# floswald/SMM.jl

Measured on AMD Instinct MI355X. Metric: chain-evals/sec (whole node), serialNormal 2p/2m, 4096 chains x 200 iters, higher is better.
Workload: dtype f64

## Files before the change

smm.jl_amd/csrc/smm_chain_persist_loc.hpp:

```cpp
#pragma once
constexpr int PL_LOCN = NORM_CT + CONE_GCAP + 2;
constexpr uint32_t PL_PBASE = ((16u * PL_LOCN + 127u) & ~127u);
constexpr int PL_HASH = 1024;
constexpr size_t PL_TSW_BASE = (size_t)8 * 8192;
constexpr int PL_TSW_TILES = 2048, PL_TSW = 8;
constexpr size_t PL_LATE_BASE = PL_TSW_BASE + (size_t)PL_TSW_TILES * (NORM_WG / 64) * PL_TSW;
constexpr int PL_LATE_N = 16384;
static_assert(PL_LATE_BASE + PL_LATE_N <= (size_t)8 * 60000, "the stamp buffer: the exchange kernels' words start at 8 * 60000");

__host__ __device__ inline size_t persist_loc_smem_bytes(const int np) {
    const size_t hw = (size_t)((H_PARAMS + 2 * np + 1) & ~1);
    const size_t dbl = (size_t)NORM_CT * np + (size_t)np * 8 * NORM_CT + (size_t)NORM_CT * persist_line(np) + 2 * 64 * (size_t)(1 + 2 * np) +
                       2 * NORM_CT * hw + (size_t)PR_ZR * 64 + 16 + 16 + 2 * 64 * 2 + (size_t)PL_LOCN * np + (size_t)PL_LOCN +
                       (size_t)(NORM_WG / 64) * PL_TSW;
    return (size_t)PL_PBASE + 2 * (size_t)CONE_LEVELS * 64 * 4 + 2 * (size_t)CONE_GCAP * 2 + 4 * 16 * 4 + 2 * (size_t)PL_HASH * 4 + dbl * 8;
}

template <int NP>
struct PersistLocLds {
    using L = NormLayout<NP>;
    static constexpr int CT = NORM_CT, RW = L::RW, HW = L::HW, LW = PR_STW + RW, RNGW = 1 + 2 * NP;
    uint32_t pbase, gbase, hbase, tbase;
    uint32_t* s_hdr;
    double *s_theta, *s_part, *s_st, *s_rng, *s_hrow, *s_xrow, *s_z0, *s_const, *s_gth, *s_thr;
    uint4* s_donor;
    unsigned long long *s_ts, *s_wts;
    unsigned* s_arrived; int* s_minprog; unsigned* s_abort; unsigned* s_xmask; int* s_glready; int* s_pub; int* s_hready;
    __device__ inline PersistLocLds(unsigned char* lds) {
        pbase = PL_PBASE;
        gbase = pbase + 2u * CONE_LEVELS * 64 * 4;
        hbase = gbase + 2u * CONE_GCAP * 2;
        tbase = hbase + 4u * 16 * 4;
        s_hdr = (uint32_t*)(lds + hbase);
        s_theta = (double*)(lds + tbase + 2u * PL_HASH * 4);
        s_part = s_theta + CT * NP;
        s_st = s_part + NP * 8 * CT;
        s_rng = s_st + CT * LW;
        s_hrow = s_rng + 2 * 64 * RNGW;
        s_xrow = s_hrow + CT * HW;
        s_z0 = s_xrow + CT * HW;
        s_const = s_z0 + PR_ZR * 64;
        s_ts = (unsigned long long*)(s_const + 16);
        s_arrived = (unsigned*)(s_ts + 8);
        s_minprog = (int*)(s_arrived + 1);
        s_abort = s_arrived + 2;
        s_xmask = s_arrived + 3;
        s_glready = (int*)(s_arrived + 4);
        s_pub = (int*)(s_arrived + 5);
        s_hready = (int*)(s_arrived + 6);
        s_donor = (uint4*)(s_const + 16 + 16);
        s_gth = s_const + 16 + 16 + 2 * 64 * 2;
        s_thr = s_gth + PL_LOCN * NP;
        s_wts = (unsigned long long*)(s_thr + PL_LOCN);
    }
};

__device__ inline uint32_t pl_hslot(const uint32_t chain) { return (chain * 2654435761u) >> 22; }
static_assert(PL_HASH == 1024, "pl_hslot: 10 bits");
__device__ inline void pl_hash_put(uint32_t* tab, const uint32_t chain, const uint32_t local) {
    uint32_t h = pl_hslot(chain);
    while (atomicCAS(&tab[h], 0u, ((chain + 1u) << 16) | local) != 0u) h = (h + 1u) & (PL_HASH - 1);
}
__device__ inline uint32_t pl_hash_get(const uint32_t* tab, const uint32_t chain) {
    uint32_t h = pl_hslot(chain);
    for (int probe = 0; probe < PL_HASH; ++probe) {
        const uint32_t v = tab[h];
        if ((v >> 16) == chain + 1u) return v & 0xffffu;
        if (v == 0u) break;
        h = (h + 1u) & (PL_HASH - 1);
    }
    return 0xffffu;
}

__device__ inline void pl_wts_add(unsigned long long* w, const unsigned long long a, const unsigned long long b, const unsigned long long c,
                                  const unsigned long long d) {
    w[0] += a; w[1] += b; w[2] += c; w[3] += d; w[5] += 1ull;
}
__device__ inline void pl_wts_out(unsigned long long* ts, const unsigned long long* w, const int tile, const int wave) {
    if (tile >= PL_TSW_TILES) return;
    unsigned long long* o = ts + PL_TSW_BASE + ((size_t)tile * (NORM_WG / 64) + (size_t)wave) * PL_TSW;
    for (int k = 0; k < PL_TSW; ++k) o[k] = k == 4 ? (unsigned long long)__builtin_amdgcn_s_getreg((31 << 11) | 4) : w[k];
}

struct PersistLocWalkValues {
    PrWait W; const uint4* ring; const uint16_t* gl; uint32_t c0g; uint32_t tag; int RW; int NPV; int t;
    __device__ __forceinline__ double value(const uint32_t s) const {
        const uint32_t g = s < (uint32_t)NORM_CT ? c0g + s : (uint32_t)gl[s - NORM_CT];
        return pr_tie_value(W, ring, nullptr, tag, RW, NPV, t, g);
    }
};

struct PlGather3 { uint4 q0, q1, q2; };
__device__ __attribute__((noinline)) PlGather3 pl_wait_gather3(const PrWait W, const uint4* p0, const uint4* p1, const uint4* p2, const uint32_t tag, const int t, const int g) {
    PlGather3 o;
    o.q0 = make_uint4(0u, 0u, 0u, 0u); o.q1 = o.q0; o.q2 = o.q0;
    if (*W.s_abort) return o;
    const unsigned long long w0 = wall_clock64();
    unsigned spins = 0;
    for (;;) {
        __builtin_amdgcn_s_sleep(2);
        p2p_u32x4 q0, q1, q2;
        asm volatile("global_load_dwordx4 %0, %3, off sc0 sc1\n\tglobal_load_dwordx4 %1, %4, off sc0 sc1\n\tglobal_load_dwordx4 %2, %5, off sc0 sc1\n\ts_waitcnt vmcnt(0)"
                     : "=&v"(q0), "=&v"(q1), "=&v"(q2) : "v"(p0), "v"(p1), "v"(p2) : "memory");
        o.q0 = make_uint4(q0.x, q0.y, q0.z, q0.w); o.q1 = make_uint4(q1.x, q1.y, q1.z, q1.w); o.q2 = make_uint4(q2.x, q2.y, q2.z, q2.w);
        if (p2p_ll_ok(o.q0, tag) && p2p_ll_ok(o.q1, tag) && p2p_ll_ok(o.q2, tag)) break;
        if ((++spins & 63u) == 0u && pr_give_up(W, w0)) { pr_abort(W, t, g); break; }
    }
    return o;
}

template <int NP, bool WIDE, bool SH, bool PCT = false>
__global__ __launch_bounds__(NORM_WG, 4) void k_chain_persist_loc(const PersistArgs A) {
    static_assert(!PCT || (WIDE && !SH), "thresholds by chain: the wide walk of a single shard");
    static_assert(NP == 1 || NP == 2, "one moment per half of the workgroup");
    extern __shared__ __attribute__((aligned(16))) unsigned char lds[];
    using LY = PersistLocLds<NP>;
    constexpr int CT = NORM_CT, RW = LY::RW, HW = LY::HW, LW = LY::LW, RNGW = LY::RNGW;
    constexpr int NPC = RW / 2, NPH = HW / 2;
    constexpr uint32_t SB = WIDE ? 16u : 8u;
    const int tid = (int)threadIdx.x, lane = tid & 63;
    const int wave = __builtin_amdgcn_readfirstlane(tid >> 6);
    const int tile = (int)blockIdx.x, tiles = (int)gridDim.x;
    const int N = A.N;
    const LY Y(lds);
    const uint32_t epoch = A.epoch;
    const int t0 = A.t0, t1 = A.t1;
    unsigned char* const mine = A.self;
    uint32_t* const pr_ctl = (uint32_t*)(mine + A.o_ctl);
    uint32_t* const pr_progress = (uint32_t*)(mine + A.o_progress);
    const PrWait W{A.err, pr_ctl, Y.s_abort, A.epoch, A.tmo};
    const int rmask = A.ring_k - 1;
    const int tiles_all = SH ? tiles * A.G : tiles;
    const uint32_t c0g = (uint32_t)(A.offset + tile * CT);
    const bool exch_any = A.Ng > 1;
    auto exch_on = [&](const int tx) { return exch_any && tx >= A.exch_from; };

    if (error_before(*(const volatile unsigned long long*)A.err, t0)) return;

    if (tid < 64) {
        const int cl = lane >> 2, r = lane & 3, c = tile * CT + cl;
        if (c < N) {
            const double2* g_cs = (const double2*)(A.cs + (size_t)c * CSW);
            const double2* g_rec = (const double2*)(A.rec_in + (size_t)c * RW);
            double2* st2 = (double2*)(Y.s_st + cl * LW);
            for (int i = r; i < 6; i += 4) st2[i] = g_cs[i];
            for (int i = r; i < NPC; i += 4) st2[PR_STW / 2 + i] = g_rec[i];
            if (r == 0) {
                const double v0 = g_rec[0].x;
                if (SH && v0 != v0) pr_report(A.err, 3, t0, (int)c0g + cl);
                if constexpr (WIDE) ((uint4*)lds)[cl] = make_uint4((uint32_t)__double2loint(v0), (uint32_t)__double2hiint(v0), (uint32_t)cl, 0u);
                else ((uint2*)lds)[cl] = make_uint2(order_key32(v0), (uint32_t)cl);
                for (int k = 0; k < NP; ++k) Y.s_gth[cl * NP + k] = A.rec_in[(size_t)c * RW + 3 + k];
                if constexpr (PCT) Y.s_thr[cl] = A.mi_g[c0g + (uint32_t)cl];
            }
        }
#pragma unroll
        for (int u = 0; u < PR_ZR; ++u) Y.s_z0[u * 64 + lane] = (lane + u * WG < A.ns) ? A.Z[lane + (size_t)u * WG] : 0.0;
    }
    if (tid >= 64 && tid < 64 + NP) {
        const int k = tid - 64;
        Y.s_const[k] = A.lb[k]; Y.s_const[NP + k] = A.ub[k]; Y.s_const[2 * NP + k] = A.mom[k]; Y.s_const[3 * NP + k] = A.w[k];
    }
    if (tid == 128) {
        Y.s_const[4 * NP] = A.failbox ? A.objp[0] : 1.0; Y.s_const[4 * NP + 1] = A.failbox ? A.objp[1] : 0.0;
        Y.s_const[4 * NP + 2] = (double)A.ns;
        *Y.s_arrived = 0u; *Y.s_minprog = 0; *Y.s_abort = 0u; *Y.s_xmask = 0u; *Y.s_glready = t0 - 2; *Y.s_pub = t0 - 2; *Y.s_hready = t0 - 2;
    }
    if (tid >= 192 && tid < 200) Y.s_ts[tid - 192] = 0ull;
    if (A.ts && tid >= 256 && tid < 256 + (NORM_WG / 64) * PL_TSW) Y.s_wts[tid - 256] = 0ull;
    if (wave == 3 && lane < CONE_HDRW) {
        if (A.walk_first) Y.s_hdr[((t0 - 1) & 3) * 16 + lane] = A.cone_hdr[((size_t)(t0 - 1 - A.plan_t0) * tiles + tile) * CONE_HDRW + lane];
        if (t0 < t1 && exch_on(t0)) Y.s_hdr[(t0 & 3) * 16 + lane] = A.cone_hdr[((size_t)(t0 - A.plan_t0) * tiles + tile) * CONE_HDRW + lane];
// ... 245 lines not shown
            if (t < t1 && exch_on(t)) request_lists(t);
            PR_BARRIER();
            unsigned long long tw0 = 0, tw1 = 0, tw2 = 0;
            if (A.ts) tw0 = wall_clock64();
            if (simw) {
                __builtin_amdgcn_s_setprio(1);
                if (nfull == PR_ZR - 1) persist_simulate<NP, true>(z, nfull, extra, Y.s_theta, Y.s_part, h, wih, A.ts != nullptr, tw1);
                else persist_simulate<NP, false>(z, nfull, extra, Y.s_theta, Y.s_part, h, wih, A.ts != nullptr, tw1);
                if (A.ts) tw2 = wall_clock64();
                __builtin_amdgcn_fence(__ATOMIC_RELEASE, "workgroup");
                const int lane3 = (int)__builtin_amdgcn_mbcnt_hi(~0u, __builtin_amdgcn_mbcnt_lo(~0u, 0u));
                if (lane3 == 0) __hip_atomic_fetch_add(Y.s_arrived, 1u, __ATOMIC_RELAXED, __HIP_MEMORY_SCOPE_WORKGROUP);
                __builtin_amdgcn_s_setprio(0);
            }
            const int lane = (int)__builtin_amdgcn_mbcnt_hi(~0u, __builtin_amdgcn_mbcnt_lo(~0u, 0u));
            const bool lists = t < t1 && exch_on(t);
            if (wave == 3 || wave >= 8) {
                if (wave == 3 && want_hdr) Y.s_hdr[((t + 1) & 3) * 16 + lane] = nhdr;
                asm volatile("s_waitcnt vmcnt(0)" ::: "memory");
                if (wave == 3 && lane == 0) __hip_atomic_store(Y.s_glready, t, __ATOMIC_RELEASE, __HIP_MEMORY_SCOPE_WORKGROUP);
                if (wave == 3 && lists) {
                    build_table(t, lane);
                    if (lane == 0) __hip_atomic_store(Y.s_hready, t, __ATOMIC_RELEASE, __HIP_MEMORY_SCOPE_WORKGROUP);
                }
                if (wave >= 8 && lists) {
                    if (!A.tables_local) while (__hip_atomic_load(Y.s_hready, __ATOMIC_ACQUIRE, __HIP_MEMORY_SCOPE_WORKGROUP) != t) __builtin_amdgcn_s_sleep(1);
                    fix_lists(t, t + 1, lane);
                }
            }
            if (wave == 2) {
                const int m = pr_min_progress(pr_progress, epoch, tiles_all, lane);
                if (lane == 0) {
                    __hip_atomic_store(Y.s_minprog, m, __ATOMIC_RELAXED, __HIP_MEMORY_SCOPE_WORKGROUP);
                    if (pr_load4_sys(pr_ctl) == epoch) *Y.s_abort = 1u;
                    if (lists && A.cone_ok[t - A.plan_t0] == 0u) pr_report(A.err, 3, t + 1, (int)c0g);
                }
                if constexpr (SH) {
                    if (*Y.s_abort && lane < A.G) {
                        unsigned char* w = nullptr;
#pragma unroll
                        for (int p = 0; p < P2P_MAXG; ++p) w = lane == p ? A.win[p] : w;
                        __hip_atomic_store((uint32_t*)(w + A.o_ctl), epoch, __ATOMIC_RELAXED, __HIP_MEMORY_SCOPE_SYSTEM);
                    }
                }
            }
            if (wave == 2 && PR_AHEAD > 1 && rng_here && t < t1) {
                const unsigned want = (unsigned)(8 * NP) * (unsigned)rel;
                while (__hip_atomic_load(Y.s_arrived, __ATOMIC_RELAXED, __HIP_MEMORY_SCOPE_WORKGROUP) < want) __builtin_amdgcn_s_sleep(2);
            }
            if ((wave == 1 || (wave == 2 && PR_AHEAD > 1)) && t < t1) make_rng(t + 1, wave - 1);
            if (wave >= 4 && wave < 8 && lists) {
                while (__hip_atomic_load(Y.s_glready, __ATOMIC_ACQUIRE, __HIP_MEMORY_SCOPE_WORKGROUP) != t) __builtin_amdgcn_s_sleep(1);
                while (__hip_atomic_load(Y.s_pub, __ATOMIC_RELAXED, __HIP_MEMORY_SCOPE_WORKGROUP) != t) __builtin_amdgcn_s_sleep(1);
                __builtin_amdgcn_s_sleep(PR_GATHER_DELAY);
                gather(t, rel, t + 1, wave * 64 + lane);
            }
            if (A.ts && lane == 0) pl_wts_add(Y.s_wts + wave * PL_TSW, tw0, tw1, tw2, wall_clock64());
        }
        PR_BARRIER();
        if (A.ts && lane == 0) pl_wts_out(A.ts, Y.s_wts + wave * PL_TSW, tile, wave);
        if (wave == 3) { store_rows(Y.s_hrow, t1, 0xffffu); store_rows(Y.s_xrow, t1 - 1, *Y.s_xmask); }
        if (wave == 1) {
            const int cl = lane >> 2, r = lane & 3, c = tile * CT + cl;
            if (c < N) {
                const double2* st2 = (const double2*)(Y.s_st + cl * LW);
                double2* g_cs = (double2*)(A.cs + (size_t)c * CSW);
                for (int i = r; i < 6; i += 4) g_cs[i] = i == 2 ? make_double2(st2[2].x, 0.0) : st2[i];
                for (int i = r; i < NPC; i += 4) ((double2*)(A.rec_out + (size_t)c * RW))[i] = st2[PR_STW / 2 + i];
                if (r == 0) {
                    const double v = Y.s_st[cl * LW + PR_STW];
                    A.vals_out[c] = v;
                    if (A.slot8_out) { A.slot8_out[c] = make_uint2(order_key32(v), (uint32_t)c); if (v != v) atomicOr(A.walk_flags, 1u); }
                }
            }
        }
        return;
    }

    const int nfull0 = A.ns / WG;
    for (int t = t0; t <= t1; ++t) {
        const int rel = t - t0 + 1;
        const bool exch = t == t0 ? A.walk_first != 0 : exch_on(t - 1);
        double z0[PR_ZR];
        PR_BARRIER();
        {
            const int lane = (int)__builtin_amdgcn_mbcnt_hi(~0u, __builtin_amdgcn_mbcnt_lo(~0u, 0u));
            const int cl = lane >> 2, r = lane & 3;
            const int c = tile * CT + cl;
            const bool valid = c < N;
            double* st = Y.s_st + cl * LW;
            unsigned long long ts1 = 0;
            if (A.ts && lane == 0) { ts1 = wall_clock64(); if (t != t0) Y.s_ts[0] += ts1 - Y.s_ts[7]; }
            uint32_t src = (uint32_t)cl;
            int partner = 0;
            const uint32_t lbase = Y.pbase + (uint32_t)((t - 1) & 1) * (CONE_LEVELS * 64 * 4);
            const uint16_t* gl = (const uint16_t*)(lds + Y.gbase) + ((t - 1) & 1) * CONE_GCAP;
            if (exch) {
                const int nsub = (int)(Y.s_hdr[((t - 1) & 3) * 16] & 0xffffu);
                if constexpr (WIDE) {
                    lean_walk_levels<64, 0, true, WalkNoGuard, PCT>(nullptr, 1, lbase, (uint32_t)(64 * lane), nsub, lane, 0, A.thr, WalkNoGuard(),
                                                                    (uint32_t)((unsigned char*)Y.s_thr - lds));
                } else {
                    const PersistLocWalkValues values{W, (const uint4*)(mine + A.o_rec) + (size_t)((rel - 1) & rmask) * A.Ng * RW, gl, c0g, pr_tag32(epoch, rel - 1), RW, NP, t};
                    lean_walk_levels<64, 0, false, PersistLocWalkValues>(nullptr, 1, lbase, (uint32_t)(64 * lane), nsub, lane, 0, 0.0, values);
                }
                if (valid) {
                    const uint32_t kmeta = WIDE ? ((const uint4*)lds)[cl].z : ((const uint2*)lds)[cl].y;
                    src = kmeta & 0xffffu;
                    if (kmeta >> 16) {
                        const uint32_t pl = lean_partner<0, WIDE ? 4 : 3>(lds, lbase, kmeta, (uint32_t)cl) - 1u;
                        partner = 1 + (int)(pl < (uint32_t)CT ? c0g + pl : (uint32_t)gl[pl - CT]);
                    }
                }
            }
            const bool donor = valid && src != (uint32_t)cl;
            const uint32_t src_g = src < (uint32_t)CT ? c0g + src : (uint32_t)gl[src - CT];
            if (donor) {
                const unsigned char* dwin = mine;
                if constexpr (SH) {
                    const int owner = (int)src_g / A.N;
#pragma unroll
                    for (int p = 0; p < P2P_MAXG; ++p) dwin = owner == p ? A.win[p] : dwin;
                }
                const uint4* g_ll = (const uint4*)(dwin + A.o_rec) + ((size_t)((rel - 1) & rmask) * A.Ng + src_g) * RW;
                const uint32_t dbase = (uint32_t)((unsigned char*)Y.s_donor - lds);
                pr_dma16(g_ll + r, dbase);
                if (4 + r < RW) pr_dma16(g_ll + 4 + r, dbase + 64 * 16);
            }
            unsigned long long ts2 = 0;
            if (A.ts && lane == 0) ts2 = wall_clock64();
            double mu01[NP], th[NP], th_old[NP];
            const double sigma = st[CS_SIGMA];
            const double* o = Y.s_rng + ((t & 1) * 64 + lane) * RNGW;
            bool found = !valid;
            {
                double x[NP];
                bool ok = valid;
#pragma unroll
                for (int k = 0; k < NP; ++k) {
                    const double lbk = Y.s_const[k], ubk = Y.s_const[NP + k];
                    th_old[k] = donor ? Y.s_gth[src * NP + k] : st[PR_STW + 3 + k];
                    th[k] = valid ? th_old[k] : 0.0;
                    mu01[k] = (th_old[k] - lbk) / (ubk - lbk);
                    const double step = sigma * o[1 + k];
                    x[k] = mu01[k] + step;
                    if (!(x[k] >= 0.0 && x[k] <= 1.0)) ok = false;
                }
                if (r >= A.smpl_iters || (A.user_n && r >= A.rb_tries)) ok = false;
                const unsigned long long m = __ballot(ok);
                const unsigned quad = (unsigned)(m >> (lane & ~3)) & 0xfu;
                if (quad) {
                    const int rwin = __builtin_ctz(quad);
#pragma unroll
                    for (int k = 0; k < NP; ++k) {
                        const double lbk = Y.s_const[k];
                        const double sc = x[k] * (Y.s_const[NP + k] - lbk);
                        const double thk = sc + lbk;
                        th[k] = quad_bcast_dyn(thk, lane, rwin);
                    }
                    found = true;
                }
            }
            if (__builtin_expect(__any(!found), 0)) {
                if (A.ts && lane == 0) Y.s_wts[7] -= wall_clock64();
                int j_next = NORM_NR;
                if (PR_AHEAD > 1 && (A.rb == nullptr || A.rb_tries >= 2 * NORM_NR)) {
                    double x[NP];
                    bool ok = !found;
#pragma unroll
                    for (int k = 0; k < NP; ++k) {
                        const double step = sigma * o[1 + NP + k];
                        x[k] = mu01[k] + step;
                        if (!(x[k] >= 0.0 && x[k] <= 1.0)) ok = false;
                    }
                    if (NORM_NR + r >= A.smpl_iters || (A.user_n && NORM_NR + r >= A.rb_tries)) ok = false;
                    const unsigned long long m = __ballot(ok);
                    const unsigned quad = (unsigned)(m >> (lane & ~3)) & 0xfu;
                    if (!found && quad) {
                        const int rwin = __builtin_ctz(quad);
#pragma unroll
                        for (int k = 0; k < NP; ++k) {
                            const double lbk = Y.s_const[k];
                            const double sc = x[k] * (Y.s_const[NP + k] - lbk);
                            const double thk = sc + lbk;
                            th[k] = quad_bcast_dyn(thk, lane, rwin);
                        }
                        found = true;
                    }
                    j_next = 2 * NORM_NR;
                }
                if (__any(!found)) {
                    const PrTries TR{A.rb, A.seed, A.rb_t0, A.N, A.RBW, A.rb_tries, A.user_n, A.smpl_iters, A.offset};
                    const PrTh<NP> lt = persist_late_tries<NP>(TR, o, t, c, valid, lane, found, sigma, mu01[0], mu01[NP - 1], Y.s_const, th[0], th[NP - 1], j_next);
#pragma unroll
                    for (int k = 0; k < NP; ++k) th[k] = lt.th[k];
                    found = lt.found;
                    if (!found && r == 0) pr_report(A.err, ERRK_NO_DRAW, t, (int)c0g + cl);
                }
                if (A.ts && lane == 0) {
                    Y.s_wts[6] += 1ull; Y.s_wts[7] += wall_clock64();
                    atomicAdd(A.ts + PL_LATE_BASE + (size_t)(t & (PL_LATE_N - 1)), 1ull);
                }
            }
            if (r == 0) {
#pragma unroll
                for (int k = 0; k < NP; ++k) Y.s_theta[cl * NP + k] = th[k];
                st[CS_PARTNER] = (double)partner;
                st[CS_WASX] = (double)src;
            }
#pragma unroll
            for (int u = 0; u < PR_ZR; ++u) z0[u] = Y.s_z0[u * 64 + lane];
            if (A.ts && lane == 0) {
                const unsigned long long ts4 = wall_clock64();
                Y.s_ts[1] += ts2 - ts1; Y.s_ts[3] += ts4 - ts2; Y.s_ts[6] = ts4;
            }
        }
        PR_BARRIER();
        unsigned long long tw0 = 0, tw1 = 0, tw2 = 0, tw3 = 0;
        if (A.ts) tw0 = wall_clock64();
        {
            const int lane_a = (int)__builtin_amdgcn_mbcnt_hi(~0u, __builtin_amdgcn_mbcnt_lo(~0u, 0u));
            const bool extra0 = lane_a < A.ns - nfull0 * WG;
            __builtin_amdgcn_s_setprio(1);
            if (nfull0 == PR_ZR - 1) persist_simulate<NP, true>(z0, nfull0, extra0, Y.s_theta, Y.s_part, 0, 0, A.ts != nullptr, tw1);
            else persist_simulate<NP, false>(z0, nfull0, extra0, Y.s_theta, Y.s_part, 0, 0, A.ts != nullptr, tw1);
            if (A.ts) tw2 = wall_clock64();
            __builtin_amdgcn_fence(__ATOMIC_RELEASE, "workgroup");
            if (lane_a == 0) __hip_atomic_fetch_add(Y.s_arrived, 1u, __ATOMIC_RELAXED, __HIP_MEMORY_SCOPE_WORKGROUP);
            __builtin_amdgcn_s_setprio(0);
        }
        {
            const unsigned want = (unsigned)(8 * NP) * (unsigned)rel;
            while (__hip_atomic_load(Y.s_arrived, __ATOMIC_RELAXED, __HIP_MEMORY_SCOPE_WORKGROUP) < want) __builtin_amdgcn_s_sleep(1);
            __builtin_amdgcn_fence(__ATOMIC_ACQUIRE, "workgroup");
        }
        if (A.ts) tw3 = wall_clock64();
        const int lane = (int)__builtin_amdgcn_mbcnt_hi(~0u, __builtin_amdgcn_mbcnt_lo(~0u, 0u));
        const int cl = lane >> 2, r = lane & 3;
        const int c = tile * CT + cl;
        const bool valid = c < N;
        double* st = Y.s_st + cl * LW;
        unsigned long long ts5 = 0;
        if (A.ts && lane == 0) ts5 = wall_clock64();
        if (valid) {
            const int src = (int)st[CS_WASX];
            const bool donor = src != cl;
            double rc2[RW];
#pragma unroll
            for (int f = 0; f < RW; ++f) rc2[f] = st[PR_STW + f];
            if (donor) {
                asm volatile("s_waitcnt vmcnt(0)" ::: "memory");
                const uint32_t tag = pr_tag32(epoch, rel - 1);
                double rr[8];
#pragma unroll
                for (int f = 0; f < 8; ++f) rr[f] = 0.0;
                bool ok = true;
#pragma unroll
                for (int f = 0; f < RW; ++f) {
                    const uint4 q = Y.s_donor[(f >> 2) * 64 + 4 * cl + (f & 3)];
                    ok = ok && p2p_ll_ok(q, tag);
                    rr[f] = p2p_ll_double(q);
                }
                if (__builtin_expect(!ok, 0)) {
                    const uint16_t* gl = (const uint16_t*)(lds + Y.gbase) + ((t - 1) & 1) * CONE_GCAP;
                    const uint32_t src_g = (uint32_t)src < (uint32_t)CT ? c0g + (uint32_t)src : (uint32_t)gl[src - CT];
                    const unsigned char* dwin = mine;
                    if constexpr (SH) {
                        const int owner = (int)src_g / A.N;
#pragma unroll
                        for (int p = 0; p < P2P_MAXG; ++p) dwin = owner == p ? A.win[p] : dwin;
                    }
                    const uint4* g_ll = (const uint4*)(dwin + A.o_rec) + ((size_t)((rel - 1) & rmask) * A.Ng + src_g) * RW;
#pragma unroll
                    for (int f = 0; f < RW; f += 2) {
                        const PrLL2 w2 = pr_wait_ll2(W, g_ll + f, g_ll + f + 1, tag, t, (int)c0g + cl);
                        rr[f] = p2p_ll_double(w2.q0); rr[f + 1] = p2p_ll_double(w2.q1);
                    }
                }
#pragma unroll
                for (int f = 0; f < RW; ++f) rc2[f] = rr[pr_ring_index<NP>(f)];
            }
            if (lane == 0) announce(rel);
            const double atun = st[CS_ATUN];
            const double uu = Y.s_rng[((t & 1) * 64 + lane) * RNGW];
            double th2[NP], sm[NP];
#pragma unroll
            for (int k = 0; k < NP; ++k) th2[k] = Y.s_theta[cl * NP + k];
            double value;
            int status;
            norm_quad_finish<NP>(in_failbox(th2[0], Y.s_const + 4 * NP), r, Y.s_part + cl, Y.s_const[4 * NP + 2],
                                 Y.s_const + 2 * NP, Y.s_const + 3 * NP, sm, value, status);
            const double old = rc2[0];
            const AcceptDecision d = accept_decide(false, status, value, old, atun, uu, pr_exp);
            if (d.negative && r == 0) pr_report(A.err, ERRK_NEGATIVE, t, (int)c0g + cl);
            const double prob = d.prob;
            const bool acc = d.acc;
            status = d.status;
            const double accd = acc ? 1.0 : 0.0;
            const double v = acc ? value : old;
            double nr[RW];
            record_head(nr, rc2, acc, value, prob, status);
#pragma unroll
            for (int k = 0; k < NP; ++k) { nr[3 + k] = acc ? th2[k] : rc2[3 + k]; nr[3 + NP + k] = acc ? sm[k] : rc2[3 + NP + k]; }
            if (RW > 3 + 2 * NP) nr[RW - 1] = 0.0;
            if (t < t1) {
// ... 69 lines not shown
```

smm.jl_amd/csrc/smm_chain_persist_tile.hpp:

```cpp
#pragma once
constexpr int PT_CT = 16;
constexpr int PT_LPC = WG / PT_CT;
constexpr int PT_NJ = 5;

struct PtLayout { uint32_t pbase, gbase, hbase, tbase, fbase, thbase, dbase; uint32_t o_cs, o_rec, o_theta, o_const, o_sm, o_vk, o_uv, o_rb, o_B; size_t total; };
__host__ __device__ inline PtLayout pt_layout(const int np, const int nm, const int RW, const int HW, const int RBW, const int kind, const int nOt, const int user_part = 0) {
    PtLayout L;
    L.pbase = PL_PBASE;
    L.gbase = L.pbase + (uint32_t)CONE_LEVELS * 64 * 4;
    L.hbase = L.gbase + (uint32_t)CONE_GCAP * 2;
    L.tbase = L.hbase + 4u * 16 * 4;
    L.fbase = L.tbase + (uint32_t)PL_HASH * 4;
    L.thbase = L.fbase + 128u;
    L.dbase = L.thbase + (uint32_t)PL_LOCN * 8u;
    uint32_t o = 0;
    L.o_cs = o; o += PT_CT * PR_STW;
    L.o_rec = o; o += 2 * PT_CT * RW;
    L.o_theta = o; o += (PT_CT * np + 1) & ~1;
    L.o_const = o; o += (2 * np + 2 * nm + 1) & ~1;
    L.o_sm = o; o += (PT_CT * nm + 1) & ~1;
    L.o_vk = o; o += (PT_CT * nm + 1) & ~1;
    L.o_uv = o; o += 2 * PT_CT;
    L.o_rb = o; o += PT_CT * RBW;
    L.o_B = o;
// ... 202 lines not shown
    auto publish = [&](const int rel, const double* rec) {
        uint4* g_ll = ring_rec(rel) + (size_t)cg * RW;
        const uint32_t tag = pr_tag32(epoch, rel);
        for (int f = r2; f < RW; f += LPC) {
            const unsigned long long a = __builtin_bit_cast(unsigned long long, rec[f]);
            const p2p_u32x4 q = {(unsigned)a, tag, (unsigned)(a >> 32), tag};
            asm volatile("global_store_dwordx4 %0, %1, off " PR_SC "\n\ts_nop 1" :: "v"(g_ll + f), "v"(q) : "memory");
            if (SH && peer_granule(f)) store_peers(rel, f, q);
        }
    };

    if (valid) {
        const double2* g_cs = (const double2*)(A.cs + (size_t)c * CSW);
        const double2* g_rec = (const double2*)(A.rec_in + (size_t)c * RW);
        for (int i = r2; i < PR_STW / 2; i += LPC) ((double2*)(s_cs + cc * PR_STW))[i] = g_cs[i];
        for (int i = r2; i < RW / 2; i += LPC) ((double2*)(s_rec + ((t0 & 1) * CT + cc) * RW))[i] = g_rec[i];
        if (r2 == 0) {
            const double v0 = A.rec_in[(size_t)c * RW];
            if (SH && v0 != v0) pr_report(A.err, 3, t0, cg);
            slots[cc] = make_uint4((uint32_t)__double2loint(v0), (uint32_t)__double2hiint(v0), (uint32_t)cc, 0u);
            if constexpr (PCT) s_thr[cc] = A.mi_g[c];
        }
    }
    for (int k = tid; k < np; k += WG) { s_lb[k] = A.lb[k]; s_ub[k] = A.ub[k]; }
    for (int k = tid; k < nm; k += WG) { s_mom[k] = A.mom[k]; s_w[k] = A.w[k]; }
    if (tid == 0) { *s_minprog = 0; *s_abort = 0u; *s_rngctr = 0u; }
    if (tid >= 64 && tid < 72) s_ts[tid - 64] = 0ull;
    if (wave == 3 && lane < CONE_HDRW) {
        if (A.walk_first) s_hdr[((t0 - 1) & 3) * 16 + lane] = A.cone_hdr[((size_t)(t0 - 1 - A.plan_t0) * tiles + tile) * CONE_HDRW + lane];
        if (t0 < t1 && exch_on(t0)) s_hdr[(t0 & 3) * 16 + lane] = A.cone_hdr[((size_t)(t0 - A.plan_t0) * tiles + tile) * CONE_HDRW + lane];
    }
    fetch_rb(t0);
    if constexpr (SH) {
        if (tile == 0 && wave == 2 && lane < A.G) {
            unsigned char* w = nullptr;
#pragma unroll
            for (int p = 0; p < P2P_MAXG; ++p) w = lane == p ? A.win[p] : w;
            __hip_atomic_store((uint32_t*)(w + A.o_arrive + 128 * (size_t)A.rank), epoch, __ATOMIC_RELAXED, __HIP_MEMORY_SCOPE_SYSTEM);
        }
        if (wave == 2) {
            const unsigned long long w0 = wall_clock64();
            unsigned spins = 0;
            bool there = lane >= A.G;
            while (__ballot(!there) != 0ull) {
                if (!there) there = (int)(__hip_atomic_load((const uint32_t*)(mine + A.o_arrive + 128 * (size_t)lane), __ATOMIC_RELAXED, __HIP_MEMORY_SCOPE_SYSTEM) - epoch) >= 0;
                if ((++spins & 63u) == 0u && (wall_clock64() - w0 > A.tmo)) {
                    if (lane == 0) { pr_report(A.err, 3, t0, (int)c0g); __hip_atomic_store(pr_ctl, epoch, __ATOMIC_RELAXED, __HIP_MEMORY_SCOPE_SYSTEM); }
                    break;
                }
                __builtin_amdgcn_s_sleep(2);
            }
        }
    }
    PR_BARRIER();
    if (SH && tid == 0 && pr_load4_sys(pr_ctl) == epoch) *s_abort = 1u;
    if (A.walk_first) {
        request_lists(t0 - 1);
        if (valid) publish(0, s_rec + ((t0 & 1) * CT + cc) * RW);
        if (wave == 2 && lane == 0 && A.cone_ok[t0 - 1 - A.plan_t0] == 0u) pr_report(A.err, 3, t0, (int)c0g);
        zero_table();
        asm volatile("s_waitcnt vmcnt(0)" ::: "memory");
        PR_BARRIER();
        build_table(t0 - 1);
        PR_BARRIER();
        fix_lists(t0 - 1, t0);
        gather(t0 - 1, 0, t0);
    }
    asm volatile("s_waitcnt vmcnt(0)" ::: "memory");
    if (!valid && r2 == 0) for (int k = 0; k < np; ++k) s_theta[cc * np + k] = 0.0;

    ZBuf zb;
    if constexpr (KIND == 1) zb.init_v(A.Z, nm, A.zstride, tid);

    for (int t = t0; t <= t1; ++t) {
        const int rel = t - t0 + 1;
        const bool exch = t == t0 ? A.walk_first != 0 : exch_on(t - 1);
        const bool lists = t < t1 && exch_on(t);
        double* const rin = s_rec + ((t & 1) * CT + cc) * RW;
        double* const rout = s_rec + (((t + 1) & 1) * CT + cc) * RW;
        PR_BARRIER();
        unsigned long long ts0 = 0;
        if (A.ts && tid == 0) { ts0 = wall_clock64(); if (t != t0) s_ts[0] += ts0 - s_ts[7]; }
        if (exch && wave == 0) {
            const int nsub = (int)(s_hdr[((t - 1) & 3) * 16] & 0xffffu);
            lean_walk_levels<64, 0, true, WalkNoGuard, PCT>(nullptr, 1, L.pbase, (uint32_t)(64 * lane), nsub, lane, 0, A.thr, WalkNoGuard(), L.thbase);
        }
        PR_BARRIER();
        unsigned long long ts1 = 0;
        if (A.ts && tid == 0) ts1 = wall_clock64();
        uint32_t src = (uint32_t)cc;
        int partner = 0;
        if (exch && valid) {
            const uint32_t kmeta = slots[cc].z;
            src = kmeta & 0xffffu;
            if (kmeta >> 16) {
                const uint32_t pl = lean_partner<0, 4>(lds, L.pbase, kmeta, (uint32_t)cc) - 1u;
                partner = 1 + (int)(pl < (uint32_t)CT ? c0g + pl : (uint32_t)gl[pl - CT]);
            }
        }
        const bool donor = valid && src != (uint32_t)cc;
        uint32_t src_g = 0u;
        if (donor) {
            src_g = src < (uint32_t)CT ? c0g + src : (uint32_t)gl[src - CT];
            const uint4* g_ll = ring_rec(rel - 1) + (size_t)src_g * RW;
            const uint32_t tag = pr_tag32(epoch, rel - 1);
            if constexpr (SH) {
                for (int f = r2; f < RW; f += LPC) {
                    if (!peer_granule(f)) continue;
                    uint4 q = pr_load16_sys(g_ll + f);
                    if (__builtin_expect(!p2p_ll_ok(q, tag), 0)) q = pt_wait_ll(W, g_ll + f, tag, t, cg);
                    rin[f] = p2p_ll_double(q);
                }
            } else if (RW <= LPC) {
                if (r2 < RW) {
                    uint4 q = pr_load16_sys(g_ll + r2);
                    if (__builtin_expect(!p2p_ll_ok(q, tag), 0)) q = pt_wait_ll(W, g_ll + r2, tag, t, cg);
                    rin[r2] = p2p_ll_double(q);
                }
            } else {
                const uint4* p[PT_NJ];
#pragma unroll
                for (int j = 0; j < PT_NJ; ++j) p[j] = g_ll + min(r2 + LPC * j, RW - 1);
                p2p_u32x4 q0, q1, q2, q3, q4;
                asm volatile("global_load_dwordx4 %0, %5, off sc0 sc1\n\tglobal_load_dwordx4 %1, %6, off sc0 sc1\n\tglobal_load_dwordx4 %2, %7, off sc0 sc1\n\t"
                             "global_load_dwordx4 %3, %8, off sc0 sc1\n\tglobal_load_dwordx4 %4, %9, off sc0 sc1\n\ts_waitcnt vmcnt(0)"
                             : "=&v"(q0), "=&v"(q1), "=&v"(q2), "=&v"(q3), "=&v"(q4) : "v"(p[0]), "v"(p[1]), "v"(p[2]), "v"(p[3]), "v"(p[4]) : "memory");
                const uint4 qq[PT_NJ] = {make_uint4(q0.x, q0.y, q0.z, q0.w), make_uint4(q1.x, q1.y, q1.z, q1.w), make_uint4(q2.x, q2.y, q2.z, q2.w),
                                         make_uint4(q3.x, q3.y, q3.z, q3.w), make_uint4(q4.x, q4.y, q4.z, q4.w)};
#pragma unroll
                for (int j = 0; j < PT_NJ; ++j) {
                    const int f = r2 + LPC * j;
                    if (f < RW) {
                        uint4 q = qq[j];
                        if (__builtin_expect(!p2p_ll_ok(q, tag), 0)) q = pt_wait_ll(W, g_ll + f, tag, t, cg);
                        rin[f] = p2p_ll_double(q);
                    }
                }
            }
        }
        if (chain_lane) s_cs[cc * PR_STW + CS_PARTNER] = (double)partner;
        PR_BARRIER();
        if (tid == 0) {
            if (!SH) __hip_atomic_store(pr_progress + tile, pr_progress_word(epoch, rel), __ATOMIC_RELAXED, __HIP_MEMORY_SCOPE_AGENT);
            *s_rngctr = 0u;
        }
        uint32_t nhdr = 0u;
        const bool want_hdr = wave == 3 && lane < CONE_HDRW && t + 1 < t1 && exch_on(t + 1);
        if (want_hdr) nhdr = A.cone_hdr[((size_t)(t + 1 - A.plan_t0) * tiles + tile) * CONE_HDRW + lane];
        if (lists) { request_lists(t); zero_table(); }
        uint32_t pw_[8] = {0xffffffffu, 0xffffffffu, 0xffffffffu, 0xffffffffu, 0xffffffffu, 0xffffffffu, 0xffffffffu, 0xffffffffu};
        uint32_t ctl_w = 0u, ok_w = 1u;
        if (wave == 2) {
#pragma unroll
            for (int j = 0; j < 8; ++j) if (lane + 64 * j < tiles_all) pw_[j] = pr_load4_sys(pr_progress + lane + 64 * j);
            if (lane == 0) { ctl_w = pr_load4_sys(pr_ctl); if (lists) ok_w = A.cone_ok[t - A.plan_t0]; }
        }
        const double uu = chain_lane ? s_rb[cc * RBW] : 0.0;
        if (chain_lane) {
            double* csb = s_cs + cc * PR_STW;
            int nn = (int)csb[CS_NNOEX], na = (int)csb[CS_NACC];
            double bp = csb[CS_BEST], bpid = csb[CS_BESTID];
            if (partner != 0) {
                const Best b = best_of(rin[0], t - 1, csb[CS_BESTP], csb[CS_BESTPID]);
                bp = b.best; bpid = b.best_id;
                if (!SH) {
                    double* hx = s_xrow + cc * HW;
                    swapped_head(hx, rin, partner, b);
                    if (HW > H_PARAMS + np + nm) hx[HW - 1] = 0.0;
// ... 260 lines not shown
```

smm.jl_amd/csrc/smm_walk_lean.hpp:

```cpp
#pragma once
__host__ __device__ inline int lean_walk_Kp(int K) { return (K + 64 * LV_MAXLEV + 3) & ~3; }
__host__ __device__ inline size_t lean_walk_bytes(int Ng, int K) { return (size_t)(((Ng + 3) & ~3) + 4) * 8 + (size_t)lean_walk_Kp(K) * 4; }
__host__ __device__ inline int lean_walk_unit(int Ng) { return 8 * (((Ng + 3) & ~3) + 2) <= 65536 ? 8 : 4; }
__host__ __device__ inline size_t lean_wide_bytes(int Ng, int K) { return (size_t)(((Ng + 3) & ~3) + 1) * 16 + (size_t)lean_walk_Kp(K) * 4; }
__host__ __device__ inline int lean_wide_unit(int Ng) { return 16 * (((Ng + 3) & ~3) + 1) <= 65536 ? 16 : 8; }
typedef unsigned int u32x4_t __attribute__((ext_vector_type(4)));
__host__ __device__ inline size_t tile_lean_slot_bytes(int Ng) { return (size_t)(((Ng + 3) & ~3) + 2) * 16; }
typedef unsigned int u32x2_t __attribute__((ext_vector_type(2)));

template <int US>
__device__ inline void lean_decode(const uint32_t pw, uint32_t& ai, uint32_t& aj) {
    if constexpr (US == 0) { ai = pw & 0xffffu; aj = pw >> 16; }
    else { ai = (pw & 0xffffu) << US; aj = (pw >> 16) << US; }
}
template <int US, int SL = 3>
__device__ inline uint32_t lean_partner(const unsigned char* lds, const uint32_t pbase, const uint32_t meta, const uint32_t g) {
    const uint32_t stamp = meta >> 16;
    if (stamp == 0u) return 0u;
    const uint32_t pw = *(const uint32_t*)(lds + pbase + 4u * (stamp - 1u));
    const uint32_t i = (pw & 0xffffu) >> (SL - US), j = (pw >> 16) >> (SL - US);
    return (i == g ? j : i) + 1u;
}

struct WalkNoGuard {};
// ... 30 lines not shown
}
__device__ inline int lean_walk_tail(const uint32_t ov, const int nlev, const int lane) {
    const uint32_t nx = (uint32_t)__shfl_down((int)ov, 1, 64);
    const unsigned long long wide = __ballot(lane < nlev && nx - ov > 64u);
    return wide ? 64 - __builtin_clzll(wide) : 0;
}
template <int NT, int US, bool WIDE = false, class GUARD = WalkNoGuard, bool PCT = false>
__device__ inline void lean_walk_levels(const double* __restrict__ vsrc, const int vstride, const uint32_t pbase, const uint32_t ov,
                                        const int nlev, const int tid, const int ltail, const double thr = 0.0, const GUARD& guard = GUARD(),
                                        const uint32_t thr_base = 0u) {
    const uint32_t wbase = (uint32_t)__builtin_amdgcn_readfirstlane(tid & ~63);
    const uint32_t tid4p = pbase + 4u * (uint32_t)tid;
    const uint32_t tidst = ((uint32_t)tid + 1u) << 16;
    uint32_t st = 0u, st1 = (uint32_t)__builtin_amdgcn_readlane((int)ov, 1);
    uint32_t pw = 0u;
    if (nlev > 0) asm volatile("ds_read_b32 %0, %1\n\ts_waitcnt lgkmcnt(0)" : "=v"(pw) : "v"(tid4p) : "memory");
    auto level = [&](const int l, const bool lone) {
        const uint32_t st2 = (uint32_t)__builtin_amdgcn_readlane((int)ov, l + 2);
        const uint32_t width = st1 - st;
        if (__builtin_expect(wbase < width, 1)) {
            uint32_t nptr;
            asm volatile("v_add_u32 %0, %1, %2" : "=v"(nptr) : "s"(st1 << 2), "v"(tid4p));
            uint32_t stamp;
            asm volatile("v_add_u32 %0, %1, %2" : "=v"(stamp) : "s"(st << 16), "v"(tidst));
            uint32_t ai, aj;
            lean_decode<US>(pw, ai, aj);
            uint32_t pwn;
            if constexpr (WIDE) {
                u32x4_t si, sj;
                double thr_l = thr;
                if constexpr (PCT)
                    asm volatile("ds_read_b128 %0, %4\n\tds_read_b128 %1, %5\n\tds_read_b32 %2, %6\n\tds_read_b64 %3, %7\n\ts_waitcnt lgkmcnt(0)"
                                 : "=&v"(si), "=&v"(sj), "=&v"(pwn), "=&v"(thr_l) : "v"(ai), "v"(aj), "v"(nptr), "v"(thr_base + (ai >> 1)) : "memory");
                else
                    asm volatile("ds_read_b128 %0, %3\n\tds_read_b128 %1, %4\n\tds_read_b32 %2, %5\n\ts_waitcnt lgkmcnt(0)"
                                 : "=&v"(si), "=&v"(sj), "=&v"(pwn) : "v"(ai), "v"(aj), "v"(nptr) : "memory");
                const double vi = __hiloint2double((int)si.y, (int)si.x), vj = __hiloint2double((int)sj.y, (int)sj.x);
                if (vi - vj > thr_l) {
                    const u32x4_t ni = {sj.x, sj.y, (sj.z & 0xffffu) | stamp, 0u}, nj = {si.x, si.y, (si.z & 0xffffu) | stamp, 0u};
                    asm volatile("ds_write_b128 %0, %2\n\tds_write_b128 %1, %3" :: "v"(ai), "v"(aj), "v"(ni), "v"(nj) : "memory");
                }
            } else {
                u32x2_t si, sj;
                asm volatile("ds_read_b64 %0, %3\n\tds_read_b64 %1, %4\n\tds_read_b32 %2, %5\n\ts_waitcnt lgkmcnt(0)"
                             : "=&v"(si), "=&v"(sj), "=&v"(pwn) : "v"(ai), "v"(aj), "v"(nptr) : "memory");
                bool swap = si.x > sj.x;
                const bool tie = si.x == sj.x;
                if (__builtin_expect(__ballot(tie) != 0ull, 0)) {
                    if (tie) swap = walk_value(guard, vsrc, vstride, si.y & 0xffffu) - walk_value(guard, vsrc, vstride, sj.y & 0xffffu) > 0.0;
                }
                if (swap) {
                    const u32x2_t ni = {sj.x, (sj.y & 0xffffu) | stamp}, nj = {si.x, (si.y & 0xffffu) | stamp};
                    asm volatile("ds_write_b64 %0, %2\n\tds_write_b64 %1, %3" :: "v"(ai), "v"(aj), "v"(ni), "v"(nj) : "memory");
                }
            }
            pw = pwn;
            if (__builtin_expect(width > (uint32_t)NT, 0)) {
                for (uint32_t o = (uint32_t)NT; wbase + o < width; o += (uint32_t)NT) {
                    uint32_t pwx;
                    asm volatile("ds_read_b32 %0, %1\n\ts_waitcnt lgkmcnt(0)" : "=v"(pwx) : "v"(tid4p + 4u * (st + o)) : "memory");
                    lean_pair<US, WIDE, GUARD, PCT>(vsrc, vstride, pwx, ((st + o) << 16) + tidst, thr, guard, thr_base);
                }
            }
        } else if (wbase < st2 - st1) {
            asm volatile("ds_read_b32 %0, %1\n\ts_waitcnt lgkmcnt(0)" : "=v"(pw) : "v"(tid4p + 4u * st1) : "memory");
        }
        st = st1; st1 = st2;
        if (!lone) { asm volatile("s_waitcnt lgkmcnt(0)" ::: "memory"); __syncthreads(); }
    };
    {
        int l = 0;
#pragma clang loop unroll(disable)
        for (; l + 2 <= ltail; l += 2) { level(l, false); level(l + 1, false); }
        if (l < ltail) level(l, false);
    }
    if (ltail < nlev && tid < 64) {
        int l = ltail;
#pragma clang loop unroll(disable)
        for (; l + 2 <= nlev; l += 2) { level(l, true); level(l + 1, true); }
        if (l < nlev) level(l, true);
        asm volatile("s_waitcnt lgkmcnt(0)" ::: "memory");
    }
}
```

Before: 334.4 million.

## Specialize single-wave exchange walk and defer donor fetch into simulate phase

Adds a dedicated single-wave (64-lane) walk routine that uses immediate LDS offsets, unrolls four sub-levels per trip and reads its header per lane with readfirstlane, replacing the generic level walker in both persist kernels. The tie-value lookup moves into a noinline cold function so the hot walk loop carries less register state. The partner lookup, donor record DMA and the CS_PARTNER/CS_WASX writes move from the exchange block into the start of the simulate block, so that work sits next to the simulation rather than before the barrier. This cuts per-level walk overhead and shortens the exchange critical path, at the cost of changing when donor data is fetched relative to its consumers.

```diff
diff --git a/smm.jl_amd/csrc/smm_chain_persist_loc.hpp b/smm.jl_amd/csrc/smm_chain_persist_loc.hpp
--- a/smm.jl_amd/csrc/smm_chain_persist_loc.hpp
+++ b/smm.jl_amd/csrc/smm_chain_persist_loc.hpp
@@ -82,12 +82,15 @@
     for (int k = 0; k < PL_TSW; ++k) o[k] = k == 4 ? (unsigned long long)__builtin_amdgcn_s_getreg((31 << 11) | 4) : w[k];
 }
 
+__device__ __attribute__((noinline, cold)) double pl_tie_value(const PrWait W, const unsigned char* win, const uint32_t o_rec, const int rel, const int rmask, const int Ng,
+                                                               const uint32_t gl, const uint32_t c0g, const int RW, const int NPV, const int t, const uint32_t s) {
+    const uint32_t g = s < (uint32_t)NORM_CT ? c0g + s : (uint32_t)*(const __attribute__((address_space(3))) uint16_t*)(size_t)(gl + 2u * (s - (uint32_t)NORM_CT));
+    const uint4* ring = (const uint4*)(win + o_rec) + (size_t)((rel - 1) & rmask) * Ng * RW;
+    return pr_tie_value(W, ring, nullptr, pr_tag32(W.epoch, rel - 1), RW, NPV, t, g);
+}
 struct PersistLocWalkValues {
-    PrWait W; const uint4* ring; const uint16_t* gl; uint32_t c0g; uint32_t tag; int RW; int NPV; int t;
-    __device__ __forceinline__ double value(const uint32_t s) const {
-        const uint32_t g = s < (uint32_t)NORM_CT ? c0g + s : (uint32_t)gl[s - NORM_CT];
-        return pr_tie_value(W, ring, nullptr, tag, RW, NPV, t, g);
-    }
+    PrWait W; const unsigned char* win; uint32_t o_rec; int rel; int rmask; int Ng; uint32_t gl; uint32_t c0g; int RW; int NPV; int t;
+    __device__ __forceinline__ double value(const uint32_t s) const { return pl_tie_value(W, win, o_rec, rel, rmask, Ng, gl, c0g, RW, NPV, t, s); }
 };
 
 struct PlGather3 { uint4 q0, q1, q2; };
@@ -499,6 +502,7 @@
         const int rel = t - t0 + 1;
         const bool exch = t == t0 ? A.walk_first != 0 : exch_on(t - 1);
         double z0[PR_ZR];
+        uint32_t wmeta;
         PR_BARRIER();
         {
             const int lane = (int)__builtin_amdgcn_mbcnt_hi(~0u, __builtin_amdgcn_mbcnt_lo(~0u, 0u));
@@ -508,42 +512,22 @@
             double* st = Y.s_st + cl * LW;
             unsigned long long ts1 = 0;
             if (A.ts && lane == 0) { ts1 = wall_clock64(); if (t != t0) Y.s_ts[0] += ts1 - Y.s_ts[7]; }
-            uint32_t src = (uint32_t)cl;
-            int partner = 0;
-            const uint32_t lbase = Y.pbase + (uint32_t)((t - 1) & 1) * (CONE_LEVELS * 64 * 4);
-            const uint16_t* gl = (const uint16_t*)(lds + Y.gbase) + ((t - 1) & 1) * CONE_GCAP;
+            wmeta = (uint32_t)cl;
             if (exch) {
-                const int nsub = (int)(Y.s_hdr[((t - 1) & 3) * 16] & 0xffffu);
+                const uint32_t lbase = Y.pbase + (uint32_t)((t - 1) & 1) * (CONE_LEVELS * 64 * 4);
+                uint32_t hw, pw0;
+                lean_sub64_head(Y.hbase + (uint32_t)((t - 1) & 3) * 64u, lbase, lane, hw, pw0);
+                const int nsub = (int)((uint32_t)__builtin_amdgcn_readfirstlane((int)hw) & 0xffffu);
                 if constexpr (WIDE) {
-                    lean_walk_levels<64, 0, true, WalkNoGuard, PCT>(nullptr, 1, lbase, (uint32_t)(64 * lane), nsub, lane, 0, A.thr, WalkNoGuard(),
-                                                                    (uint32_t)((unsigned char*)Y.s_thr - lds));
+                    lean_walk_sub64<0, true, WalkNoGuard, PCT>(lbase, nsub, lane, pw0, A.thr, WalkNoGuard(), (uint32_t)((unsigned char*)Y.s_thr - lds));
                 } else {
-                    const PersistLocWalkValues values{W, (const uint4*)(mine + A.o_rec) + (size_t)((rel - 1) & rmask) * A.Ng * RW, gl, c0g, pr_tag32(epoch, rel - 1), RW, NP, t};
-                    lean_walk_levels<64, 0, false, PersistLocWalkValues>(nullptr, 1, lbase, (uint32_t)(64 * lane), nsub, lane, 0, 0.0, values);
-                }
-                if (valid) {
-                    const uint32_t kmeta = WIDE ? ((const uint4*)lds)[cl].z : ((const uint2*)lds)[cl].y;
-                    src = kmeta & 0xffffu;
-                    if (kmeta >> 16) {
-                        const uint32_t pl = lean_partner<0, WIDE ? 4 : 3>(lds, lbase, kmeta, (uint32_t)cl) - 1u;
-                        partner = 1 + (int)(pl < (uint32_t)CT ? c0g + pl : (uint32_t)gl[pl - CT]);
-                    }
-                }
-            }
+                    const PersistLocWalkValues values{W, mine, A.o_rec, rel, rmask, A.Ng, Y.gbase + (uint32_t)((t - 1) & 1) * (CONE_GCAP * 2), c0g, RW, NP, t};
+                    lean_walk_sub64<0, false, PersistLocWalkValues>(lbase, nsub, lane, pw0, 0.0, values);
+                }
+                if (valid) wmeta = WIDE ? ((const uint4*)lds)[cl].z : ((const uint2*)lds)[cl].y;
+            }
+            const uint32_t src = wmeta & 0xffffu;
             const bool donor = valid && src != (uint32_t)cl;
-            const uint32_t src_g = src < (uint32_t)CT ? c0g + src : (uint32_t)gl[src - CT];
-            if (donor) {
-                const unsigned char* dwin = mine;
-                if constexpr (SH) {
-                    const int owner = (int)src_g / A.N;
-#pragma unroll
-                    for (int p = 0; p < P2P_MAXG; ++p) dwin = owner == p ? A.win[p] : dwin;
-                }
-                const uint4* g_ll = (const uint4*)(dwin + A.o_rec) + ((size_t)((rel - 1) & rmask) * A.Ng + src_g) * RW;
-                const uint32_t dbase = (uint32_t)((unsigned char*)Y.s_donor - lds);
-                pr_dma16(g_ll + r, dbase);
-                if (4 + r < RW) pr_dma16(g_ll + 4 + r, dbase + 64 * 16);
-            }
             unsigned long long ts2 = 0;
             if (A.ts && lane == 0) ts2 = wall_clock64();
             double mu01[NP], th[NP], th_old[NP];
@@ -622,11 +606,7 @@
             if (r == 0) {
 #pragma unroll
                 for (int k = 0; k < NP; ++k) Y.s_theta[cl * NP + k] = th[k];
-                st[CS_PARTNER] = (double)partner;
-                st[CS_WASX] = (double)src;
-            }
-#pragma unroll
-            for (int u = 0; u < PR_ZR; ++u) z0[u] = Y.s_z0[u * 64 + lane];
+            }
             if (A.ts && lane == 0) {
                 const unsigned long long ts4 = wall_clock64();
                 Y.s_ts[1] += ts2 - ts1; Y.s_ts[3] += ts4 - ts2; Y.s_ts[6] = ts4;
@@ -638,6 +618,38 @@
         {
             const int lane_a = (int)__builtin_amdgcn_mbcnt_hi(~0u, __builtin_amdgcn_mbcnt_lo(~0u, 0u));
             const bool extra0 = lane_a < A.ns - nfull0 * WG;
+#pragma unroll
+            for (int u = 0; u < PR_ZR; ++u) z0[u] = Y.s_z0[u * 64 + lane_a];
+            {
+                const int cl = lane_a >> 2, r = lane_a & 3;
+                const bool valid = tile * CT + cl < N;
+                const uint32_t src = wmeta & 0xffffu;
+                const uint32_t lbase = Y.pbase + (uint32_t)((t - 1) & 1) * (CONE_LEVELS * 64 * 4);
+                const uint16_t* gl = (const uint16_t*)(lds + Y.gbase) + ((t - 1) & 1) * CONE_GCAP;
+                int partner = 0;
+                if (wmeta >> 16) {
+                    const uint32_t pl = lean_partner<0, WIDE ? 4 : 3>(lds, lbase, wmeta, (uint32_t)cl) - 1u;
+                    partner = 1 + (int)(pl < (uint32_t)CT ? c0g + pl : (uint32_t)gl[pl - CT]);
+                }
+                if (valid && src != (uint32_t)cl) {
+                    const uint32_t src_g = src < (uint32_t)CT ? c0g + src : (uint32_t)gl[src - CT];
+                    const unsigned char* dwin = mine;
+                    if constexpr (SH) {
+                        const int owner = (int)src_g / A.N;
+#pragma unroll
+                        for (int p = 0; p < P2P_MAXG; ++p) dwin = owner == p ? A.win[p] : dwin;
+                    }
+                    const uint4* g_ll = (const uint4*)(dwin + A.o_rec) + ((size_t)((rel - 1) & rmask) * A.Ng + src_g) * RW;
+                    const uint32_t dbase = (uint32_t)((unsigned char*)Y.s_donor - lds);
+                    pr_dma16(g_ll + r, dbase);
+                    if (4 + r < RW) pr_dma16(g_ll + 4 + r, dbase + 64 * 16);
+                }
+                if (r == 0) {
+                    double* st = Y.s_st + cl * LW;
+                    st[CS_PARTNER] = (double)partner;
+                    st[CS_WASX] = (double)src;
+                }
+            }
             __builtin_amdgcn_s_setprio(1);
             if (nfull0 == PR_ZR - 1) persist_simulate<NP, true>(z0, nfull0, extra0, Y.s_theta, Y.s_part, 0, 0, A.ts != nullptr, tw1);
             else persist_simulate<NP, false>(z0, nfull0, extra0, Y.s_theta, Y.s_part, 0, 0, A.ts != nullptr, tw1);
diff --git a/smm.jl_amd/csrc/smm_chain_persist_tile.hpp b/smm.jl_amd/csrc/smm_chain_persist_tile.hpp
--- a/smm.jl_amd/csrc/smm_chain_persist_tile.hpp
+++ b/smm.jl_amd/csrc/smm_chain_persist_tile.hpp
@@ -308,8 +308,10 @@
         unsigned long long ts0 = 0;
         if (A.ts && tid == 0) { ts0 = wall_clock64(); if (t != t0) s_ts[0] += ts0 - s_ts[7]; }
         if (exch && wave == 0) {
-            const int nsub = (int)(s_hdr[((t - 1) & 3) * 16] & 0xffffu);
-            lean_walk_levels<64, 0, true, WalkNoGuard, PCT>(nullptr, 1, L.pbase, (uint32_t)(64 * lane), nsub, lane, 0, A.thr, WalkNoGuard(), L.thbase);
+            uint32_t hw, pw0;
+            lean_sub64_head(L.hbase + (uint32_t)((t - 1) & 3) * 64u, L.pbase, lane, hw, pw0);
+            const int nsub = (int)((uint32_t)__builtin_amdgcn_readfirstlane((int)hw) & 0xffffu);
+            lean_walk_sub64<0, true, WalkNoGuard, PCT>(L.pbase, nsub, lane, pw0, A.thr, WalkNoGuard(), L.thbase);
         }
         PR_BARRIER();
         unsigned long long ts1 = 0;
diff --git a/smm.jl_amd/csrc/smm_walk_lean.hpp b/smm.jl_amd/csrc/smm_walk_lean.hpp
--- a/smm.jl_amd/csrc/smm_walk_lean.hpp
+++ b/smm.jl_amd/csrc/smm_walk_lean.hpp
@@ -136,3 +136,77 @@
         asm volatile("s_waitcnt lgkmcnt(0)" ::: "memory");
     }
 }
+
+__device__ inline void lean_sub64_head(const uint32_t hoff, const uint32_t pbase, const int lane, uint32_t& hdr, uint32_t& pw) {
+    asm volatile("ds_read_b32 %0, %2\n\tds_read_b32 %1, %3\n\ts_waitcnt lgkmcnt(0)" : "=&v"(hdr), "=&v"(pw) : "v"(hoff), "v"(pbase + 4u * (uint32_t)lane) : "memory");
+}
+#define LEAN_SUB64_OFF(o) " offset:" #o "\n\t"
+template <int US, bool WIDE, class GUARD, bool PCT, int OFF>
+__device__ __forceinline__ void lean_sub64_level(const uint32_t ptr, const uint32_t stamp, uint32_t& pw, const double thr, const GUARD& guard, const uint32_t thr_base) {
+    static_assert(OFF == 256 || OFF == 512 || OFF == 768 || OFF == 1024, "the word of the next sub-level within a trip of four");
+    uint32_t ai, aj;
+    lean_decode<US>(pw, ai, aj);
+    uint32_t pwn;
+    if constexpr (WIDE) {
+        u32x4_t si, sj;
+        double thr_l = thr;
+#define LEAN_SUB64_WIDE(o) \
+        if constexpr (PCT)  \
+            asm volatile("ds_read_b128 %0, %4\n\tds_read_b128 %1, %5\n\tds_read_b32 %2, %6" LEAN_SUB64_OFF(o) "ds_read_b64 %3, %7\n\ts_waitcnt lgkmcnt(0)" \
+                         : "=&v"(si), "=&v"(sj), "=&v"(pwn), "=&v"(thr_l) : "v"(ai), "v"(aj), "v"(ptr), "v"(thr_base + (ai >> 1)) : "memory"); \
+        else \
+            asm volatile("ds_read_b128 %0, %3\n\tds_read_b128 %1, %4\n\tds_read_b32 %2, %5" LEAN_SUB64_OFF(o) "s_waitcnt lgkmcnt(0)" \
+                         : "=&v"(si), "=&v"(sj), "=&v"(pwn) : "v"(ai), "v"(aj), "v"(ptr) : "memory")
+        if constexpr (OFF == 256) { LEAN_SUB64_WIDE(256); } else if constexpr (OFF == 512) { LEAN_SUB64_WIDE(512); }
+        else if constexpr (OFF == 768) { LEAN_SUB64_WIDE(768); } else { LEAN_SUB64_WIDE(1024); }
+#undef LEAN_SUB64_WIDE
+        const double vi = __hiloint2double((int)si.y, (int)si.x), vj = __hiloint2double((int)sj.y, (int)sj.x);
+        if (vi - vj > thr_l) {
+            const u32x4_t ni = {sj.x, sj.y, (sj.z & 0xffffu) | stamp, 0u}, nj = {si.x, si.y, (si.z & 0xffffu) | stamp, 0u};
+            asm volatile("ds_write_b128 %0, %2\n\tds_write_b128 %1, %3" :: "v"(ai), "v"(aj), "v"(ni), "v"(nj) : "memory");
+        }
+    } else {
+        u32x2_t si, sj;
+#define LEAN_SUB64_KEY(o) \
+        asm volatile("ds_read_b64 %0, %3\n\tds_read_b64 %1, %4\n\tds_read_b32 %2, %5" LEAN_SUB64_OFF(o) "s_waitcnt lgkmcnt(0)" \
+                     : "=&v"(si), "=&v"(sj), "=&v"(pwn) : "v"(ai), "v"(aj), "v"(ptr) : "memory")
+        if constexpr (OFF == 256) { LEAN_SUB64_KEY(256); } else if constexpr (OFF == 512) { LEAN_SUB64_KEY(512); }
+        else if constexpr (OFF == 768) { LEAN_SUB64_KEY(768); } else { LEAN_SUB64_KEY(1024); }
+#undef LEAN_SUB64_KEY
+        bool swap = si.x > sj.x;
+        const bool tie = si.x == sj.x;
+        if (__builtin_expect(__ballot(tie) != 0ull, 0)) {
+            if (tie) swap = walk_value(guard, nullptr, 1, si.y & 0xffffu) - walk_value(guard, nullptr, 1, sj.y & 0xffffu) > 0.0;
+        }
+        if (swap) {
+            const u32x2_t ni = {sj.x, (sj.y & 0xffffu) | stamp}, nj = {si.x, (si.y & 0xffffu) | stamp};
+            asm volatile("ds_write_b64 %0, %2\n\tds_write_b64 %1, %3" :: "v"(ai), "v"(aj), "v"(ni), "v"(nj) : "memory");
+        }
+    }
+    pw = pwn;
+}
+#undef LEAN_SUB64_OFF
+template <int US, bool WIDE = false, class GUARD = WalkNoGuard, bool PCT = false>
+__device__ inline void lean_walk_sub64(const uint32_t pbase, const int nsub, const int lane, uint32_t pw, const double thr = 0.0, const GUARD& guard = GUARD(),
+                                       const uint32_t thr_base = 0u) {
+    static_assert(!std::is_same<GUARD, WalkNoGuard>::value || WIDE, "a key tie reads the exact values through the guard: there is no plain array here");
+    constexpr uint32_t SUBST = 64u << 16;
+    uint32_t ptr = pbase + 4u * (uint32_t)lane;
+    uint32_t stamp = ((uint32_t)lane + 1u) << 16;
+    int left = nsub;
+#pragma clang loop unroll(disable)
+    for (; left >= 4; left -= 4) {
+        lean_sub64_level<US, WIDE, GUARD, PCT, 256>(ptr, stamp, pw, thr, guard, thr_base);
+        lean_sub64_level<US, WIDE, GUARD, PCT, 512>(ptr, stamp + SUBST, pw, thr, guard, thr_base);
+        lean_sub64_level<US, WIDE, GUARD, PCT, 768>(ptr, stamp + 2u * SUBST, pw, thr, guard, thr_base);
+        lean_sub64_level<US, WIDE, GUARD, PCT, 1024>(ptr, stamp + 3u * SUBST, pw, thr, guard, thr_base);
+        ptr += 1024u; stamp += 4u * SUBST;
+    }
+    if (left & 2) {
+        lean_sub64_level<US, WIDE, GUARD, PCT, 256>(ptr, stamp, pw, thr, guard, thr_base);
+        lean_sub64_level<US, WIDE, GUARD, PCT, 512>(ptr, stamp + SUBST, pw, thr, guard, thr_base);
+        ptr += 512u; stamp += 2u * SUBST;
+    }
+    if (left & 1) lean_sub64_level<US, WIDE, GUARD, PCT, 256>(ptr, stamp, pw, thr, guard, thr_base);
+    asm volatile("s_waitcnt lgkmcnt(0)" ::: "memory");
+}
```

Measured after the change: 361.8 million (median of 6 runs). +8.2%, better.
